# yjh0410/YOLO-Nano

Measured on NVIDIA B200. Metric: images/sec YOLO-Nano-1.0x 416 bs256 fp32-parity e2e (backbone+neck+head+decode+NMS), higher is better.
Workload: dtype f32 (tcgen05 3xTF32 split, fp32 accumulate)

## Files before the change

### yolo_nano_b200/csrc/ptx_sm100.cuh

```cuda
#pragma once
#include <cuda.h>
#include <cuda_runtime.h>
#include <stdint.h>

namespace ynb {
namespace ptx {

__device__ __forceinline__ uint32_t smem_u32(const void* p) {
  return (uint32_t)__cvta_generic_to_shared(p);
}

__device__ __forceinline__ void mbar_init(uint64_t* bar, uint32_t count) {
  asm volatile("mbarrier.init.shared::cta.b64 [%0], %1;" ::"r"(smem_u32(bar)), "r"(count));
}
__device__ __forceinline__ void fence_barrier_init() {
  asm volatile("fence.mbarrier_init.release.cluster;" ::: "memory");
}
__device__ __forceinline__ void mbar_arrive(uint64_t* bar) {
  asm volatile("mbarrier.arrive.shared::cta.b64 _, [%0];" ::"r"(smem_u32(bar)) : "memory");
}
__device__ __forceinline__ void mbar_arrive_expect_tx(uint64_t* bar, uint32_t bytes) {
  asm volatile("mbarrier.arrive.expect_tx.shared::cta.b64 _, [%0], %1;" ::"r"(smem_u32(bar)), "r"(bytes)
               : "memory");
}
// ... 26 lines not shown
  }
  if (timeout_flag) atomicCAS(timeout_flag, 0, code);
  return false;
}

__device__ __forceinline__ void fence_proxy_async_smem() {
  asm volatile("fence.proxy.async.shared::cta;" ::: "memory");
}
__device__ __forceinline__ void tc_fence_before_sync() {
  asm volatile("tcgen05.fence::before_thread_sync;" ::: "memory");
}
__device__ __forceinline__ void tc_fence_after_sync() {
  asm volatile("tcgen05.fence::after_thread_sync;" ::: "memory");
}

__device__ __forceinline__ void prefetch_tmap(const CUtensorMap* m) {
  asm volatile("prefetch.tensormap [%0];" ::"l"(reinterpret_cast<uint64_t>(m)) : "memory");
}
__device__ __forceinline__ void tma_load_2d(void* smem_dst, const CUtensorMap* m, uint64_t* bar, int c0, int c1) {
  asm volatile(
      "cp.async.bulk.tensor.2d.shared::cluster.global.mbarrier::complete_tx::bytes [%0], [%1, {%3, %4}], [%2];"
      ::"r"(smem_u32(smem_dst)), "l"(reinterpret_cast<uint64_t>(m)), "r"(smem_u32(bar)), "r"(c0), "r"(c1)
      : "memory");
}
__device__ __forceinline__ void tma_load_4d(void* smem_dst, const CUtensorMap* m, uint64_t* bar, int c0, int c1,
                                            int c2, int c3) {
  asm volatile(
      "cp.async.bulk.tensor.4d.shared::cluster.global.mbarrier::complete_tx::bytes [%0], [%1, {%3, %4, %5, %6}], [%2];"
      ::"r"(smem_u32(smem_dst)), "l"(reinterpret_cast<uint64_t>(m)), "r"(smem_u32(bar)), "r"(c0), "r"(c1),
      "r"(c2), "r"(c3)
      : "memory");
}

__device__ __forceinline__ void tma_prefetch_4d(const CUtensorMap* m, int c0, int c1, int c2, int c3) {
  asm volatile("cp.async.bulk.prefetch.tensor.4d.L2.global.tile [%0, {%1, %2, %3, %4}];"
               ::"l"(reinterpret_cast<uint64_t>(m)), "r"(c0), "r"(c1), "r"(c2), "r"(c3)
               : "memory");
}

__device__ __forceinline__ void cp_async_16(void* smem_dst, const void* gsrc, uint32_t src_bytes) {
  asm volatile("cp.async.cg.shared.global [%0], [%1], 16, %2;" ::"r"(smem_u32(smem_dst)), "l"(gsrc), "r"(src_bytes)
               : "memory");
}
__device__ __forceinline__ void cp_async_commit() { asm volatile("cp.async.commit_group;" ::: "memory"); }
__device__ __forceinline__ void cp_async_wait_all() { asm volatile("cp.async.wait_group 0;" ::: "memory"); }

__device__ __forceinline__ void tma_store_2d(const CUtensorMap* m, const void* smem_src, int c0, int c1) {
  asm volatile("cp.async.bulk.tensor.2d.global.shared::cta.bulk_group [%0, {%2, %3}], [%1];"
               ::"l"(reinterpret_cast<uint64_t>(m)), "r"(smem_u32(smem_src)), "r"(c0), "r"(c1)
               : "memory");
}
__device__ __forceinline__ void tma_store_4d(const CUtensorMap* m, const void* smem_src, int c0, int c1, int c2, int c3) {
  asm volatile("cp.async.bulk.tensor.4d.global.shared::cta.bulk_group [%0, {%2, %3, %4, %5}], [%1];"
               ::"l"(reinterpret_cast<uint64_t>(m)), "r"(smem_u32(smem_src)), "r"(c0), "r"(c1), "r"(c2), "r"(c3)
               : "memory");
}
__device__ __forceinline__ void bulk_commit() { asm volatile("cp.async.bulk.commit_group;" ::: "memory"); }
template <int N>
__device__ __forceinline__ void bulk_wait_read() {
  asm volatile("cp.async.bulk.wait_group.read %0;" ::"n"(N) : "memory");
}
template <int N>
__device__ __forceinline__ void bulk_wait() {
  asm volatile("cp.async.bulk.wait_group %0;" ::"n"(N) : "memory");
}

// ... 99 lines not shown
```

### yolo_nano_b200/csrc/unit_tc.cuh

```cuda
#pragma once
#include "gemm_tc.cuh"

namespace ynb {

constexpr int kDpThreads = 640;
constexpr int kDpEpiWarps = 8;
constexpr int kDpDwWarp0 = 8, kDpDwWarps = 8;
constexpr int kDpRawWarp = 16, kDpMmaWarp = 17, kDpWWarp = 18;
constexpr int kDpMaxAStages = 4, kDpMaxRawStages = 4;
constexpr int kDpStgBytes = kDpEpiWarps * 4096;

struct DwPwParams {
  int H, W, lgTW, tiles_x, tiles_y;
  int64_t num_tiles;
  int C4;
  int num_chunks;
  int ksub;
  int N, Npad;
  int mode;
  int w_resident, a_stages, raw_stages;
  int prefetch_tiles;
  int pass_blocks;
  int tma_out;
  uint32_t tmem_cols;
  const float* dw_w;
  const float* dw_b;
  int dw_act;
  float* out;
  int out_ld, out_off;
  ChanMap omap;
  const float* bias;
  int act;
  const float* pass;
  int pass_ld;
  int* err_flag;
  long long* trace;
};

#define YNB_DP_TRACE(role, lt, kc)                                                              \
  do {                                                                                           \
    if (p.trace != nullptr && blockIdx.x == 0 && (lt) < 16)                                      \
      p.trace[((role) * 16 + (lt)) * 8 + ((kc) & 7)] = clock64();                               \
  } while (0)

struct DpSmemLayout {
  uint32_t raw_stride, a_off, a_stride, w_chunk_bytes, w_res_off, dww_off, bias_off, stg_off, bar_off, total;
};

__host__ __device__ inline DpSmemLayout dp_smem_layout(int Npad, int num_chunks, int lgTW, int a_stages, int raw_stages,
                                                       bool w_resident, bool split, int chunk_ch = 32) {
  DpSmemLayout L;
  const int TW = 1 << lgTW, TH = kTcBM >> lgTW;
  L.w_chunk_bytes = (uint32_t)Npad * 128;
  L.raw_stride = ((uint32_t)((TW + 2) * (TH + 2) * 128) + 1023u) & ~1023u;
  L.a_off = L.raw_stride * raw_stages;
  L.a_stride = kTcAStageBytes * (split ? 2 : 1) + (w_resident ? 0 : L.w_chunk_bytes * (split ? 2 : 1));
  L.w_res_off = L.a_off + L.a_stride * a_stages;
  const uint32_t w_res = w_resident ? L.w_chunk_bytes * (split ? 2 : 1) * num_chunks : 0;
  L.dww_off = L.w_res_off + w_res;
  L.bias_off = L.dww_off + (((uint32_t)(10 * num_chunks * chunk_ch * 4) + 1023u) & ~1023u);
  L.stg_off = L.bias_off + 1024;
  L.bar_off = L.stg_off + kDpStgBytes;
  L.total = L.bar_off + 256 + 1024;
  return L;
}

__device__ __forceinline__ float cvt_rna_tf32(float x) {
  uint32_t r;
  asm("cvt.rna.tf32.f32 %0, %1;" : "=r"(r) : "f"(x));
  return __uint_as_float(r);
}

template <bool kPass, typename E>
__global__ void __launch_bounds__(kDpThreads, 1)
dwpw_tc_kernel(const __grid_constant__ CUtensorMap tmIn, const __grid_constant__ CUtensorMap tmWhi,
               const __grid_constant__ CUtensorMap tmWlo, const __grid_constant__ CUtensorMap tmPass,
               const __grid_constant__ CUtensorMap tmOut, const DwPwParams p) {
  extern __shared__ __align__(16) uint8_t smem_raw[];
  uint8_t* smem = smem_raw + ((1024u - (ptx::smem_u32(smem_raw) & 1023u)) & 1023u);

  constexpr bool kBf16 = sizeof(E) == 2;
  constexpr int CH = 128 / (int)sizeof(E);
  constexpr int CGS = CH / 4;
  const bool split = !kBf16 && p.mode == YNB_GEMM_TC_3XTF32;
  const DpSmemLayout lay = dp_smem_layout(p.Npad, p.num_chunks, p.lgTW, p.a_stages, p.raw_stages, p.w_resident != 0, split, CH);
  const uint32_t w_chunk_bytes = lay.w_chunk_bytes;
  const int KC = p.num_chunks * CH;
  const int TW = 1 << p.lgTW, TH = kTcBM >> p.lgTW;
  float* s_dww = reinterpret_cast<float*>(smem + lay.dww_off);
  float* s_bias = reinterpret_cast<float*>(smem + lay.bias_off);
  uint64_t* bars = reinterpret_cast<uint64_t*>(smem + lay.bar_off);
  uint64_t* raw_full = bars;
  uint64_t* raw_empty = bars + 4;
  uint64_t* a_ready = bars + 8;
  uint64_t* a_empty = bars + 12;
  uint64_t* w_full = bars + 16;
  uint64_t* tmem_full = bars + 20;
  uint64_t* tmem_empty = bars + 22;
  uint32_t* tmem_ptr = reinterpret_cast<uint32_t*>(bars + 24);

  const int warp = threadIdx.x >> 5, lane = threadIdx.x & 31;
  pdl_trigger();

  if (warp == kDpRawWarp && lane == 0) {
    ptx::prefetch_tmap(&tmIn);
    ptx::prefetch_tmap(&tmWhi);
    if (split) ptx::prefetch_tmap(&tmWlo);
    if (p.pass_blocks) ptx::prefetch_tmap(&tmPass);
    if (p.tma_out) ptx::prefetch_tmap(&tmOut);
    for (int s = 0; s < kDpMaxRawStages; ++s) {
      ptx::mbar_init(&raw_full[s], 1);
      ptx::mbar_init(&raw_empty[s], kBf16 ? kDpDwWarps : kDpDwWarps / 2);
    }
    for (int s = 0; s < kDpMaxAStages; ++s) {
      ptx::mbar_init(&a_ready[s], kBf16 ? kDpDwWarps : kDpDwWarps / 2);
      ptx::mbar_init(&a_empty[s], 1);
      ptx::mbar_init(&w_full[s], 1);
    }
// ... 9 lines not shown
  }
  for (int i = threadIdx.x; i < 10 * KC; i += kDpThreads) {
    const int tap = i / KC, c = i - tap * KC;
    float v = 0.0f;
    if (c < p.C4) v = tap < 9 ? __ldg(p.dw_w + tap * p.C4 + c) : __ldg(p.dw_b + c);
    s_dww[i] = v;
  }
  for (int i = threadIdx.x; i < p.Npad; i += kDpThreads) s_bias[i] = i < p.N ? __ldg(p.bias + i) : 0.0f;
  ptx::tc_fence_before_sync();
  __syncthreads();
  ptx::tc_fence_after_sync();
  const uint32_t tmem_base = *tmem_ptr;

  const int nacc = split ? 2 : 1;
  const int acc_cols = p.Npad * nacc;
  const int per_img = p.tiles_x * p.tiles_y;
  auto a_stage = [&](int s) { return smem + lay.a_off + (size_t)s * lay.a_stride; };
  auto w_hi_ptr = [&](int s, int kc) {
    return p.w_resident ? smem + lay.w_res_off + (size_t)kc * w_chunk_bytes * (split ? 2 : 1)
                        : a_stage(s) + kTcAStageBytes * (split ? 2 : 1);
  };

  if (warp == kDpRawWarp && p.w_resident && ptx::elect_one()) {
    ptx::mbar_arrive_expect_tx(&w_full[0], w_chunk_bytes * (split ? 2 : 1) * p.num_chunks);
    for (int kc = 0; kc < p.num_chunks; ++kc) {
      ptx::tma_load_2d(w_hi_ptr(0, kc), &tmWhi, &w_full[0], kc * CH, 0);
      if (split) ptx::tma_load_2d(w_hi_ptr(0, kc) + w_chunk_bytes, &tmWlo, &w_full[0], kc * CH, 0);
    }
  }
  pdl_wait();

  if (warp == kDpRawWarp) {
    if (ptx::elect_one()) {
      const uint32_t raw_bytes = (uint32_t)((TW + 2) * (TH + 2) * 128);
      int r = 0;
      uint32_t ph = 0;
      bool ok = true;
      for (int64_t tile = blockIdx.x; tile < p.num_tiles && ok; tile += gridDim.x) {
        const int b = (int)(tile / per_img);
        const int rr = (int)(tile - (int64_t)b * per_img);
        const int y0 = (rr / p.tiles_x) * TH, x0 = (rr % p.tiles_x) * TW;
#pragma unroll 1
        for (int cb = 0; cb < p.pass_blocks; ++cb) ptx::tma_prefetch_4d(&tmPass, cb * CH, x0, y0, b);
        if (p.prefetch_tiles > 0) {
          const int64_t tp = tile + (int64_t)p.prefetch_tiles * gridDim.x;
          if (tp < p.num_tiles) {
            const int bp = (int)(tp / per_img);
            const int rp = (int)(tp - (int64_t)bp * per_img);
            const int yp = (rp / p.tiles_x) * TH, xp = (rp % p.tiles_x) * TW;
#pragma unroll 1
            for (int kc = 0; kc < p.num_chunks; ++kc) ptx::tma_prefetch_4d(&tmIn, kc * CH, xp - 1, yp - 1, bp);
          }
        }
        for (int kc = 0; kc < p.num_chunks; ++kc) {
          ok = ptx::mbar_wait(&raw_empty[r], ph ^ 1, p.err_flag, 1);
          if (!ok) break;
          ptx::mbar_arrive_expect_tx(&raw_full[r], raw_bytes);
          ptx::tma_load_4d(smem + (size_t)r * lay.raw_stride, &tmIn, &raw_full[r], kc * CH, x0 - 1, y0 - 1, b);
          YNB_DP_TRACE(0, (int)((tile - blockIdx.x) / gridDim.x), kc);
          if (++r == p.raw_stages) { r = 0; ph ^= 1; }
        }
      }
    }
  } else if (warp == kDpWWarp) {
    if (!p.w_resident && ptx::elect_one()) {
      int s = 0;
      uint32_t ph = 0;
      bool ok = true;
      for (int64_t tile = blockIdx.x; tile < p.num_tiles && ok; tile += gridDim.x) {
        for (int kc = 0; kc < p.num_chunks; ++kc) {
          ok = ptx::mbar_wait(&a_empty[s], ph ^ 1, p.err_flag, 2);
// ... 34 lines not shown
          for (int k = 0; k < kTcBK / 8; ++k) {
            if (k >= nk) break;
            const uint32_t ko = k * 32;
            const uint32_t accum = (kc | k) != 0;
            const uint64_t da = ptx::make_sw128_kmajor_desc(a_hi + ko);
            const uint64_t db = ptx::make_sw128_kmajor_desc(b_hi + ko);
            if (kBf16) {
              ptx::mma_bf16_ss(d_tmem, da, db, idesc, accum);
            } else if (stack_b) {
              ptx::mma_tf32_ss(d_tmem, da, db, idesc2, accum);
              ptx::mma_tf32_ss(c_tmem, ptx::make_sw128_kmajor_desc(a_lo + ko), db, idesc, 1);
            } else if (split) {
              ptx::mma_tf32_ss(c_tmem, ptx::make_sw128_kmajor_desc(a_lo + ko), db, idesc, accum);
              ptx::mma_tf32_ss(c_tmem, da, ptx::make_sw128_kmajor_desc(b_lo + ko), idesc, 1);
              ptx::mma_tf32_ss(d_tmem, da, db, idesc, accum);
            } else {
              ptx::mma_tf32_ss(d_tmem, da, db, idesc, accum);
            }
          }
          YNB_DP_TRACE(3, (int)((tile - blockIdx.x) / gridDim.x), kc);
          ptx::mma_commit(&a_empty[s]);
          if (kc == p.num_chunks - 1) ptx::mma_commit(&tmem_full[acc]);
          if (++s == p.a_stages) { s = 0; ph ^= 1; }
        }
        if (++acc == 2) { acc = 0; acc_ph ^= 1; }
      }
    }
  } else if (warp >= kDpDwWarp0 && warp < kDpDwWarp0 + kDpDwWarps) {
    constexpr int NGROUPS = kBf16 ? 1 : 2;
    constexpr int GTHREADS = 256 / NGROUPS;
    const int t = (threadIdx.x - kDpDwWarp0 * 32) % GTHREADS;
    const int grp = (threadIdx.x - kDpDwWarp0 * 32) / GTHREADS;
    const int cg = t & (CGS - 1);
    const int IW = TW + 2;
    const bool has_act = p.dw_act != YNB_ACT_NONE;
    const float slope = p.dw_act == YNB_ACT_RELU ? 0.0f : 0.1f;
    const int nloc = (int64_t)blockIdx.x < p.num_tiles
                         ? (int)((p.num_tiles - blockIdx.x + gridDim.x - 1) / gridDim.x) : 0;
    const int total_chunks = nloc * p.num_chunks;
    bool ok = true;
    {
      for (int gc = grp; gc < total_chunks && ok; gc += NGROUPS) {
        const int lt_ = gc / p.num_chunks, kc = gc - lt_ * p.num_chunks;
        const int r = gc % p.raw_stages, s = gc % p.a_stages;
        const uint32_t rph = (uint32_t)((gc / p.raw_stages) & 1), sph = (uint32_t)((gc / p.a_stages) & 1);
        const float* wv = s_dww + kc * CH + cg * 4;
        const float4 bv = *reinterpret_cast<const float4*>(wv + 9 * KC);
        ok = ptx::mbar_wait(&raw_full[r], rph, p.err_flag, 7);
        if (ok) ok = ptx::mbar_wait(&a_empty[s], sph ^ 1, p.err_flag, 8);
        if (!ok) break;
        if (t == 0) YNB_DP_TRACE(1, lt_, kc);
        const uint8_t* raw = smem + (size_t)r * lay.raw_stride;
        uint8_t* a_hi = a_stage(s);
        uint8_t* a_lo = a_hi + kTcAStageBytes;
        constexpr int ROWS = 2;
        const int bidx = t / CGS;
        const int nsx = TW >> 2;
        const int sx = bidx % nsx, sy = (bidx / nsx) * ROWS;
        float4 acc[ROWS][4];
#pragma unroll
        for (int o = 0; o < ROWS; ++o)
#pragma unroll
          for (int q = 0; q < 4; ++q) acc[o][q] = bv;
#pragma unroll
        for (int ir = 0; ir < ROWS + 2; ++ir) {
          const int r0 = (sy + ir) * IW + sx * 4;
          float4 v[6];
#pragma unroll
          for (int j = 0; j < 6; ++j) {
            const int rr = r0 + j;
            if (!kBf16) v[j] = load4(reinterpret_cast<const E*>(raw + rr * 128 + (cg << 4)));
            else v[j] = load4(reinterpret_cast<const E*>(raw + rr * 128 + (cg << 3)));
          }
#pragma unroll
          for (int o = 0; o < ROWS; ++o) {
            const int ky = ir - o;
            if (ky < 0 || ky > 2) continue;
#pragma unroll
            for (int kx = 0; kx < 3; ++kx) {
              const float4 k = *reinterpret_cast<const float4*>(wv + (ky * 3 + kx) * KC);
#pragma unroll
              for (int q = 0; q < 4; ++q) {
                const float4 u = v[q + kx];
                const float2 lo = __ffma2_rn(make_float2(u.x, u.y), make_float2(k.x, k.y), make_float2(acc[o][q].x, acc[o][q].y));
                const float2 hi = __ffma2_rn(make_float2(u.z, u.w), make_float2(k.z, k.w), make_float2(acc[o][q].z, acc[o][q].w));
                acc[o][q] = make_float4(lo.x, lo.y, hi.x, hi.y);
              }
            }
          }
        }
        __syncwarp();
        if (lane == 0) ptx::mbar_arrive(&raw_empty[r]);
#pragma unroll
        for (int o = 0; o < ROWS; ++o) {
          const int row0 = (sy + o) * TW + sx * 4;
#pragma unroll
          for (int q = 0; q < 4; ++q) {
            const int row = row0 + q;
            float4 a = acc[o][q];
            if (has_act) {
              a.x = fmaxf(a.x, a.x * slope); a.y = fmaxf(a.y, a.y * slope);
              a.z = fmaxf(a.z, a.z * slope); a.w = fmaxf(a.w, a.w * slope);
            }
            if (kBf16) {
              const uint32_t o2 = (uint32_t)row * 128 + ((uint32_t)((cg >> 1) ^ (row & 7)) << 4) + ((uint32_t)(cg & 1) << 3);
              *reinterpret_cast<uint2*>(a_hi + o2) = make_uint2(pack_bf16x2(a.x, a.y), pack_bf16x2(a.z, a.w));
            } else {
              const uint32_t o2 = (uint32_t)row * 128 + ((uint32_t)(cg ^ (row & 7)) << 4);
              if (split) {
                float4 h, l;
                h.x = cvt_rna_tf32(a.x); h.y = cvt_rna_tf32(a.y); h.z = cvt_rna_tf32(a.z); h.w = cvt_rna_tf32(a.w);
                l.x = cvt_rna_tf32(a.x - h.x); l.y = cvt_rna_tf32(a.y - h.y);
                l.z = cvt_rna_tf32(a.z - h.z); l.w = cvt_rna_tf32(a.w - h.w);
                *reinterpret_cast<float4*>(a_hi + o2) = h;
                *reinterpret_cast<float4*>(a_lo + o2) = l;
              } else {
                *reinterpret_cast<float4*>(a_hi + o2) = a;
              }
            }
          }
        }
        ptx::fence_proxy_async_smem();
        __syncwarp();
        if (lane == 0) ptx::mbar_arrive(&a_ready[s]);
        if (t == 0) YNB_DP_TRACE(2, lt_, kc);
      }
    }
  } else if (warp < kDpEpiWarps) {
    const int group = warp >> 2, q = warp & 3;
    const int row = q * 32 + lane;
    const float slope = p.act == YNB_ACT_RELU ? 0.0f : (p.act == YNB_ACT_LEAKY ? 0.1f : 1.0f);
    uint8_t* sbox = smem + lay.stg_off + warp * 4096;
    const int sw = lane & 7;
    const int yy = row >> p.lgTW, xx = row & (TW - 1);
    const bool gap = p.omap.gap != 0;
    constexpr int BOX = 128 / (int)sizeof(E);
    constexpr int CPB = kPass ? BOX / 2 : BOX;
    constexpr int EPC = 16 / (int)sizeof(E);
    const int nbox = (p.Npad + CPB - 1) / CPB;
    const int out_cols = kPass ? 2 * p.N : ((p.N + EPC - 1) / EPC) * EPC;
    E* const outp = reinterpret_cast<E*>(p.out);
    const E* const passp = reinterpret_cast<const E*>(p.pass);
    const int acc = group;
    bool ok = true;
    int lt = group;
    for (int64_t tile = blockIdx.x + (int64_t)group * gridDim.x; tile < p.num_tiles && ok; tile += 2 * (int64_t)gridDim.x, lt += 2) {
      const uint32_t acc_ph = (uint32_t)((lt >> 1) & 1);
      const int b = (int)(tile / per_img);
      const int rr = (int)(tile - (int64_t)b * per_img);
      const int y = (rr / p.tiles_x) * TH + yy, x = (rr % p.tiles_x) * TW + xx;
      const bool valid = y < p.H && x < p.W;
      const int pix = (b * p.H + y) * p.W + x;
      const int ooff = valid ? pix * p.out_ld : -1;
      const E* prow = passp + (valid ? (size_t)pix * p.pass_ld : 0);
      uint4 x1v[4];
      auto fetch_x1 = [&](int c0) {
#pragma unroll
        for (int j = 0; j < 4; ++j)
          x1v[j] = (kPass && valid && c0 + EPC * j < p.N) ? __ldg(reinterpret_cast<const uint4*>(prow + c0) + j)
                                                         : make_uint4(0u, 0u, 0u, 0u);
      };
      if (kPass) fetch_x1(0);
      ok = ptx::mbar_wait(&tmem_full[acc], acc_ph, p.err_flag, 9);
      if (!ok) break;
      ptx::tc_fence_after_sync();
      if (q == 0 && lane == 0) YNB_DP_TRACE(4, lt, 0);
      const uint32_t t_base = tmem_base + ((uint32_t)(q * 32) << 16) + (uint32_t)(acc * acc_cols);
      auto drain16 = [&](int c0, float (&v)[16]) {
        uint32_t r1[16];
        ptx::tmem_ld_32x16(t_base + c0, r1);
        if (nacc == 2) {
          uint32_t r2[16];
          ptx::tmem_ld_32x16(t_base + (uint32_t)p.Npad + c0, r2);
          ptx::tmem_ld_wait();
#pragma unroll
          for (int j = 0; j < 16; ++j) v[j] = __uint_as_float(r1[j]) + __uint_as_float(r2[j]);
        } else {
          ptx::tmem_ld_wait();
#pragma unroll
          for (int j = 0; j < 16; ++j) v[j] = __uint_as_float(r1[j]);
        }
#pragma unroll
        for (int j = 0; j < 4; ++j) {
          const float4 b4 = *reinterpret_cast<const float4*>(s_bias + c0 + 4 * j);
          v[4 * j] += b4.x; v[4 * j + 1] += b4.y; v[4 * j + 2] += b4.z; v[4 * j + 3] += b4.w;
// ... 58 lines not shown
                const uint32_t x1bits = (i & 1) ? (xs >> 16) : (xs & 0xffffu);
                w[i] = x1bits | (pack_bf16x2(0.0f, v[i]) & 0xffff0000u);
              }
#pragma unroll
              for (int j = 0; j < 4; ++j) put_chunk(4 * h + j, make_uint4(w[4 * j], w[4 * j + 1], w[4 * j + 2], w[4 * j + 3]));
            }
          }
        } else {
          box_free();
#pragma unroll
          for (int h = 0; h < 4; ++h) {
            if (h == 0 || c0 + 16 * h < p.Npad) {
              float v[16];
              drain16(c0 + 16 * h, v);
              put_chunk(2 * h, make_uint4(pack_bf16x2(v[0], v[1]), pack_bf16x2(v[2], v[3]), pack_bf16x2(v[4], v[5]),
                                          pack_bf16x2(v[6], v[7])));
              put_chunk(2 * h + 1, make_uint4(pack_bf16x2(v[8], v[9]), pack_bf16x2(v[10], v[11]), pack_bf16x2(v[12], v[13]),
                                              pack_bf16x2(v[14], v[15])));
            }
          }
        }
        if (kPass && bx + 1 < nbox) fetch_x1((bx + 1) * CPB);
        if (bx == nbox - 1) {
          ptx::tc_fence_before_sync();
          __syncwarp();
          if (lane == 0) ptx::mbar_arrive(&tmem_empty[acc]);
        }
        __syncwarp();
        const int j0 = bx * BOX;
        if (tma_out) {
          ptx::fence_proxy_async_smem();
          __syncwarp();
          if (ptx::elect_one()) {
            ptx::tma_store_4d(&tmOut, sbox, j0, (rr % p.tiles_x) * TW, (rr / p.tiles_x) * TH + q * (32 >> p.lgTW), b);
            ptx::bulk_commit();
          }
          continue;
        }
        if (!gap) {
          const int ch = lane & 7;
          const int jc = j0 + EPC * ch;
#pragma unroll
          for (int k = 0; k < 8; ++k) {
            const int r = (lane >> 3) + 4 * k;
            const int oo = __shfl_sync(0xffffffffu, ooff, r);
            const uint4 val = *reinterpret_cast<const uint4*>(sbox + r * 128 + ((ch ^ (r & 7)) << 4));
            if (oo >= 0 && jc < out_cols) *reinterpret_cast<uint4*>(outp + oo + p.out_off + jc) = val;
          }
        } else if (!kBf16) {
          const int pr = lane & 15;
          const int jc = j0 + 2 * pr;
          const int col = p.omap.slot(p.out_off + jc);
#pragma unroll
          for (int k = 0; k < 16; ++k) {
            const int r = (lane >> 4) + 2 * k;
            const int oo = __shfl_sync(0xffffffffu, ooff, r);
            const uint2 val =
                *reinterpret_cast<const uint2*>(sbox + r * 128 + ((((pr >> 1) ^ (r & 7)) << 4) | ((pr & 1) << 3)));
            if (oo >= 0 && jc < out_cols) *reinterpret_cast<uint2*>(outp + oo + col) = val;
          }
        } else {
          const int jc = j0 + 2 * lane;
          const int col = p.omap.slot(p.out_off + jc);
#pragma unroll 8
          for (int r = 0; r < 32; ++r) {
            const int oo = __shfl_sync(0xffffffffu, ooff, r);
            const uint32_t val =
// ... 5 lines not shown
      }
      if (q == 0 && lane == 0) YNB_DP_TRACE(5, lt, 0);
    }
    if (p.tma_out && ptx::elect_one()) ptx::bulk_wait<0>();
  }

  ptx::tc_fence_before_sync();
  __syncthreads();
  if (warp == kDpMmaWarp) {
    ptx::tc_fence_after_sync();
    ptx::tmem_dealloc(tmem_base, p.tmem_cols);
  }
}

struct DwPwLaunch {
  CUtensorMap tmIn;
  CUtensorMap tmOut;
  CUtensorMap tmPass;
  const TcWeights* w = nullptr;
  DwPwParams p;
  uint32_t smem = 0;
  unsigned grid = 0;
};

inline bool plan_dwpw(DwPwLaunch& L, const void* in, int in_ld, int B, int H, int W, int C, int C4, const TcWeights* w,
                      int mode) {
  DwPwParams& p = L.p;
  const bool split = mode == YNB_GEMM_TC_3XTF32;
  const bool is_bf16 = mode == YNB_GEMM_TC_BF16;
  const int es = is_bf16 ? 2 : 4, chunk_ch = 128 / es;
  if (2 * (split ? 2 : 1) * w->Npad > 512 || (reinterpret_cast<uintptr_t>(in) & 15u) || ((in_ld * es) & 15)) return false;
  if ((int64_t)B * H * W * std::max(p.out_ld, std::max(p.pass_ld, 1)) >= (1LL << 31)) return false;
  p.H = H; p.W = W;
  {
    const int t16 = ((W + 15) / 16) * ((H + 7) / 8), t32 = ((W + 31) / 32) * ((H + 3) / 4);
    p.lgTW = t32 < t16 ? 5 : 4;
    static const int force = getenv("YNB_DP_LGTW") ? atoi(getenv("YNB_DP_LGTW")) : 0;
    if (force == 4 || force == 5) p.lgTW = force;
  }
  const int TW = 1 << p.lgTW, TH = kTcBM >> p.lgTW;
  p.tiles_x = (W + TW - 1) / TW;
  p.tiles_y = (H + TH - 1) / TH;
  p.num_tiles = (int64_t)B * p.tiles_x * p.tiles_y;
  p.C4 = C4;
  p.num_chunks = w->Kpad / chunk_ch;
  p.ksub = (C * es + 31) / 32;
  p.N = w->N; p.Npad = w->Npad;
  p.mode = mode;
  p.tmem_cols = 32;
  while ((int)p.tmem_cols < 2 * (split ? 2 : 1) * p.Npad) p.tmem_cols <<= 1;
  bool found = false;
  static const int wres = getenv("YNB_DP_WRES") ? atoi(getenv("YNB_DP_WRES")) : -1;
  for (int raw = kDpMaxRawStages; raw >= 2 && !found; --raw)
    for (int resident = 1; resident >= 0 && !found; --resident) {
      if (wres >= 0 && resident != wres) continue;
      DpSmemLayout lay = dp_smem_layout(p.Npad, p.num_chunks, p.lgTW, 2, raw, resident != 0, split, chunk_ch);
      if (lay.total <= (uint32_t)kTcSmemBudget) {
        p.a_stages = 2; p.raw_stages = raw; p.w_resident = resident; L.smem = lay.total;
        found = true;
      }
    }
  if (!found) return false;
  {
    static const int pf = getenv("YNB_DP_PREFETCH") ? atoi(getenv("YNB_DP_PREFETCH")) : 0;
    p.prefetch_tiles = pf;
  }
  const int epc = 16 / es;
  if ((reinterpret_cast<uintptr_t>(p.out) & 15u) || (p.out_ld % epc) || (p.out_off % epc)) return false;
  p.pass_blocks = 0;
  if (p.pass) {
    if ((reinterpret_cast<uintptr_t>(p.pass) & 15u) || (p.pass_ld % epc)) return false;
    if (make_tmap_nhwc(&L.tmPass, p.pass, (p.N + epc - 1) / epc * epc, W, H, B, p.pass_ld, TW, TH, is_bf16))
      p.pass_blocks = (p.N + chunk_ch - 1) / chunk_ch;
  }
  if (!make_tmap_nhwc(&L.tmIn, in, C4, W, H, B, in_ld, TW + 2, TH + 2, is_bf16, false)) return false;
  p.tma_out = 0;
  {
    static const bool no_ts = getenv("YNB_DP_NO_TMA_STORE") != nullptr;
    const int out_cols = p.pass ? 2 * p.N : (p.N + epc - 1) / epc * epc;
    if (!no_ts && p.omap.gap == 0 && p.out_off == 0 &&
        make_tmap_nhwc(&L.tmOut, p.out, out_cols, W, H, B, p.out_ld, TW, 32 / TW, is_bf16))
      p.tma_out = 1;
  }
  L.w = w;
  L.grid = (unsigned)std::min<int64_t>(p.num_tiles, kNumSMs);
  return true;
}

inline cudaError_t launch_dwpw_tc(const DwPwLaunch& L, cudaStream_t st) {
  using KernelT = void (*)(CUtensorMap, CUtensorMap, CUtensorMap, CUtensorMap, CUtensorMap, DwPwParams);
  static const KernelT kernels[4] = {dwpw_tc_kernel<false, float>, dwpw_tc_kernel<true, float>,
                                     dwpw_tc_kernel<false, bf16>, dwpw_tc_kernel<true, bf16>};
  static bool attr_set = false;
  if (!attr_set) {
    for (KernelT k : kernels) {
      cudaError_t e = cudaFuncSetAttribute(k, cudaFuncAttributeMaxDynamicSharedMemorySize, kTcSmemBudget);
      if (e != cudaSuccess) return e;
    }
    attr_set = true;
  }
  const int ki = (L.p.mode == YNB_GEMM_TC_BF16 ? 2 : 0) + (L.p.pass != nullptr ? 1 : 0);
  cudaError_t r = launch_pdl(kernels[ki], dim3(L.grid), dim3(kDpThreads), (size_t)L.smem, st,
                             L.tmIn, L.w->tm_hi, L.w->tm_lo, L.p.pass_blocks ? L.tmPass : L.tmIn,
                             L.p.tma_out ? L.tmOut : L.tmIn, L.p);
  YNB_COUNT_LAUNCH();
  return r;
}

}
```

### yolo_nano_b200/csrc/ynb_api.cu

```cuda
#include <cuda.h>
#include <cuda_runtime.h>

#include <cmath>
#include <cstdio>
#include <cstdlib>
#include <cstring>
#include <deque>
#include <functional>
#include <map>
#include <memory>
#include <string>
#include <tuple>
#include <vector>

#include "yolonano_b200.h"

#include "common.cuh"
#include "decode_nms.cuh"
#include "nms_grid.cuh"
#include "gemm_ffma.cuh"
#include "gemm_tc.cuh"
#include "unit_tc.cuh"
#include "kernels_basic.cuh"
#include "train_ops.cuh"
// ... 1611 lines not shown
  UNIT_TRY(cudaMemcpy(t.hi, hi.data(), hi.size() * 4, cudaMemcpyHostToDevice));
  UNIT_TRY(cudaMemcpy(t.lo, lo.data(), lo.size() * 4, cudaMemcpyHostToDevice));
  if (bfm) UNIT_TRY(cudaMemcpy(t.hi, bwv.data(), bwv.size() * 2, cudaMemcpyHostToDevice));
  int rc = YNB_OK;
  DwPwLaunch L;
  DwPwParams& p = L.p;
  memset(&p, 0, sizeof(p));
  p.dw_w = dw_w; p.dw_b = dw_b; p.dw_act = dw_act;
  p.out = out; p.out_ld = out_ld; p.out_off = 0; p.omap = dense_map();
  p.bias = pw_b; p.act = act; p.pass = pass; p.pass_ld = pass ? pass_ld : 0; p.err_flag = d_err;
  long long* d_trace = nullptr;
  const bool want_trace = getenv("YNB_DP_TRACE") != nullptr;
  if (want_trace) {
    UNIT_TRY(cudaMalloc(&d_trace, 6 * 16 * 8 * 8));
    UNIT_TRY(cudaMemset(d_trace, 0, 6 * 16 * 8 * 8));
    p.trace = d_trace;
  }
  if (!make_tmap_2d(&t.tm_hi, t.hi, t.Kpad, t.Npad, t.Kpad, t.Npad, bfm) ||
      !make_tmap_2d(&t.tm_lo, t.lo, t.Kpad, t.Npad, t.Kpad, t.Npad) ||
      !plan_dwpw(L, in, in_ld, batch, h, w_, channels, channels, &t, mode)) {
    rc = fail(nullptr, YNB_ERR_CUDA, "ynb_dwpw_tc: tensor map / smem planning failed");
  } else {
    cudaError_t r = launch_dwpw_tc(L, st);
    if (r == cudaSuccess) r = cudaStreamSynchronize(st);
    int flag = 0;
    if (r == cudaSuccess) r = cudaMemcpy(&flag, d_err, 4, cudaMemcpyDeviceToHost);
    if (r != cudaSuccess) rc = fail(nullptr, YNB_ERR_CUDA, std::string("ynb_dwpw_tc: ") + cudaGetErrorString(r));
    else if (flag) rc = fail(nullptr, YNB_ERR_CUDA, "ynb_dwpw_tc: mbarrier timeout code " + std::to_string(flag));
    if (want_trace && r == cudaSuccess) {
      std::vector<long long> h(6 * 16 * 8);
      cudaMemcpy(h.data(), d_trace, h.size() * 8, cudaMemcpyDeviceToHost);
      long long t0 = 0;
      for (long long v : h) if (v && (!t0 || v < t0)) t0 = v;
      fprintf(stderr, "YNB_DP_TRACE chunks=%d a_stages=%d raw_stages=%d resident=%d lgTW=%d tiles=%lld grid=%u\n", L.p.num_chunks,
              L.p.a_stages, L.p.raw_stages, L.p.w_resident, L.p.lgTW, (long long)L.p.num_tiles, L.grid);
      const char* names[6] = {"raw_issued", "raw_landed", "A_written", "mma_issued", "acc_ready", "epi_done"};
      for (int lt = 0; lt < 16; ++lt)
        for (int role = 0; role < 6; ++role) {
          std::string line;
          for (int kc = 0; kc < 8; ++kc)
            if (h[(role * 16 + lt) * 8 + kc]) line += " " + std::to_string(h[(role * 16 + lt) * 8 + kc] - t0);
          if (!line.empty()) fprintf(stderr, "TRACE tile %2d %-11s%s\n", lt, names[role], line.c_str());
        }
    }
  }
  if (d_trace) cudaFree(d_trace);
  cudaFree(t.hi); cudaFree(t.lo); cudaFree(d_err);
  return rc;
}

YNB_EXPORT int ynb_stem_pool(const float* x, float* out, const float* w, const float* b, int32_t batch,
                             int32_t input_size, void* stream) {
  if (!x || !out || !w || !b || input_size % 32) return fail(nullptr, YNB_ERR_INVALID, "ynb_stem_pool: bad arguments");
  StemWeights wt;
  UNIT_TRY(cudaMemcpy(wt.w, w, sizeof(wt.w), cudaMemcpyDeviceToHost));
  UNIT_TRY(cudaMemcpy(wt.b, b, sizeof(wt.b), cudaMemcpyDeviceToHost));
  CUtensorMap tmx{};
  const int use_tma = make_tmap_stem_input(&tmx, x, input_size, batch) ? 1 : 0;
  UNIT_TRY(launch_stem_pool(x, out, false, wt, tmx, use_tma, batch, input_size, (cudaStream_t)stream));
  return YNB_OK;
}

YNB_EXPORT int ynb_decode_level(const float* raw, int32_t raw_ld, float* boxes, float* scores, int32_t* cls,
                                int32_t batch, int32_t grid, int32_t stride_px, int32_t input_size,
                                const float* anchors_wh, int32_t num_anchors, int32_t num_classes,
                                int64_t boxes_per_image, int64_t level_off, void* stream) {
  if (!raw || !boxes || !scores || !cls || !anchors_wh || num_anchors > 4)
    return fail(nullptr, YNB_ERR_INVALID, "ynb_decode_level: bad arguments");
// ... 717 lines not shown
```

Measured before the change: 35230.

## Add flat pixel tiling to fused depthwise+pointwise tensor-core kernel

Adds a flat tiling mode in which each tile covers 128 consecutive pixels across the flattened B*H*W space, replacing 2D rectangular tiles when W is small enough. Raw input is loaded as a single 2D TMA box holding the tile plus one halo row above and below. Border taps are masked with per-thread bitmasks, and output and pass stores use 2D tensor maps. The goal is to remove the padding waste of rectangular tiles on small or odd feature maps and cut tile count. In exchange it adds halo rows spanning full image width, larger raw smem stages, and extra per-tap branching in the depthwise loop.

After: 35240, median of 6. No clear change (+0.0%).

```diff
diff --git a/yolo_nano_b200/csrc/ptx_sm100.cuh b/yolo_nano_b200/csrc/ptx_sm100.cuh
--- a/yolo_nano_b200/csrc/ptx_sm100.cuh
+++ b/yolo_nano_b200/csrc/ptx_sm100.cuh
@@ -82,6 +82,11 @@
       : "memory");
 }
 
+__device__ __forceinline__ void tma_prefetch_2d(const CUtensorMap* m, int c0, int c1) {
+  asm volatile("cp.async.bulk.prefetch.tensor.2d.L2.global.tile [%0, {%1, %2}];"
+               ::"l"(reinterpret_cast<uint64_t>(m)), "r"(c0), "r"(c1)
+               : "memory");
+}
 __device__ __forceinline__ void tma_prefetch_4d(const CUtensorMap* m, int c0, int c1, int c2, int c3) {
   asm volatile("cp.async.bulk.prefetch.tensor.4d.L2.global.tile [%0, {%1, %2, %3, %4}];"
                ::"l"(reinterpret_cast<uint64_t>(m)), "r"(c0), "r"(c1), "r"(c2), "r"(c3)
diff --git a/yolo_nano_b200/csrc/unit_tc.cuh b/yolo_nano_b200/csrc/unit_tc.cuh
--- a/yolo_nano_b200/csrc/unit_tc.cuh
+++ b/yolo_nano_b200/csrc/unit_tc.cuh
@@ -12,6 +12,8 @@
 
 struct DwPwParams {
   int H, W, lgTW, tiles_x, tiles_y;
+  int flat;
+  int P;
   int64_t num_tiles;
   int C4;
   int num_chunks;
@@ -47,12 +49,17 @@
   uint32_t raw_stride, a_off, a_stride, w_chunk_bytes, w_res_off, dww_off, bias_off, stg_off, bar_off, total;
 };
 
-__host__ __device__ inline DpSmemLayout dp_smem_layout(int Npad, int num_chunks, int lgTW, int a_stages, int raw_stages,
-                                                       bool w_resident, bool split, int chunk_ch = 32) {
+constexpr int kDpFlatMaxW = (256 - kTcBM - 2) / 2;
+__host__ __device__ inline uint32_t dp_raw_box_bytes(int flat, int lgTW, int W) {
+  if (flat) return (uint32_t)(kTcBM + 2 * W + 2) * 128u;
+  return (uint32_t)(((1 << lgTW) + 2) * ((kTcBM >> lgTW) + 2) * 128);
+}
+
+__host__ __device__ inline DpSmemLayout dp_smem_layout(int Npad, int num_chunks, int flat, int lgTW, int W, int a_stages,
+                                                       int raw_stages, bool w_resident, bool split, int chunk_ch = 32) {
   DpSmemLayout L;
-  const int TW = 1 << lgTW, TH = kTcBM >> lgTW;
   L.w_chunk_bytes = (uint32_t)Npad * 128;
-  L.raw_stride = ((uint32_t)((TW + 2) * (TH + 2) * 128) + 1023u) & ~1023u;
+  L.raw_stride = (dp_raw_box_bytes(flat, lgTW, W) + 1023u) & ~1023u;
   L.a_off = L.raw_stride * raw_stages;
   L.a_stride = kTcAStageBytes * (split ? 2 : 1) + (w_resident ? 0 : L.w_chunk_bytes * (split ? 2 : 1));
   L.w_res_off = L.a_off + L.a_stride * a_stages;
@@ -83,7 +90,8 @@
   constexpr int CH = 128 / (int)sizeof(E);
   constexpr int CGS = CH / 4;
   const bool split = !kBf16 && p.mode == YNB_GEMM_TC_3XTF32;
-  const DpSmemLayout lay = dp_smem_layout(p.Npad, p.num_chunks, p.lgTW, p.a_stages, p.raw_stages, p.w_resident != 0, split, CH);
+  const DpSmemLayout lay =
+      dp_smem_layout(p.Npad, p.num_chunks, p.flat, p.lgTW, p.W, p.a_stages, p.raw_stages, p.w_resident != 0, split, CH);
   const uint32_t w_chunk_bytes = lay.w_chunk_bytes;
   const int KC = p.num_chunks * CH;
   const int TW = 1 << p.lgTW, TH = kTcBM >> p.lgTW;
@@ -159,11 +167,31 @@
 
   if (warp == kDpRawWarp) {
     if (ptx::elect_one()) {
-      const uint32_t raw_bytes = (uint32_t)((TW + 2) * (TH + 2) * 128);
+      const uint32_t raw_bytes = dp_raw_box_bytes(p.flat, p.lgTW, p.W);
       int r = 0;
       uint32_t ph = 0;
       bool ok = true;
-      for (int64_t tile = blockIdx.x; tile < p.num_tiles && ok; tile += gridDim.x) {
+      for (int64_t tile = blockIdx.x; tile < p.num_tiles && ok && p.flat; tile += gridDim.x) {
+        const int p0 = (int)tile * kTcBM;
+#pragma unroll 1
+        for (int cb = 0; cb < p.pass_blocks; ++cb) ptx::tma_prefetch_2d(&tmPass, cb * CH, p0);
+        if (p.prefetch_tiles > 0) {
+          const int64_t tp = tile + (int64_t)p.prefetch_tiles * gridDim.x;
+          if (tp < p.num_tiles) {
+#pragma unroll 1
+            for (int kc = 0; kc < p.num_chunks; ++kc) ptx::tma_prefetch_2d(&tmIn, kc * CH, (int)tp * kTcBM - p.W - 1);
+          }
+        }
+        for (int kc = 0; kc < p.num_chunks; ++kc) {
+          ok = ptx::mbar_wait(&raw_empty[r], ph ^ 1, p.err_flag, 1);
+          if (!ok) break;
+          ptx::mbar_arrive_expect_tx(&raw_full[r], raw_bytes);
+          ptx::tma_load_2d(smem + (size_t)r * lay.raw_stride, &tmIn, &raw_full[r], kc * CH, p0 - p.W - 1);
+          YNB_DP_TRACE(0, (int)((tile - blockIdx.x) / gridDim.x), kc);
+          if (++r == p.raw_stages) { r = 0; ph ^= 1; }
+        }
+      }
+      for (int64_t tile = blockIdx.x; tile < p.num_tiles && ok && !p.flat; tile += gridDim.x) {
         const int b = (int)(tile / per_img);
         const int rr = (int)(tile - (int64_t)b * per_img);
         const int y0 = (rr / p.tiles_x) * TH, x0 = (rr % p.tiles_x) * TW;
@@ -264,20 +292,30 @@
     const int t = (threadIdx.x - kDpDwWarp0 * 32) % GTHREADS;
     const int grp = (threadIdx.x - kDpDwWarp0 * 32) / GTHREADS;
     const int cg = t & (CGS - 1);
-    const int IW = TW + 2;
-    const bool has_act = p.dw_act != YNB_ACT_NONE;
-    const float slope = p.dw_act == YNB_ACT_RELU ? 0.0f : 0.1f;
-    const int nloc = (int64_t)blockIdx.x < p.num_tiles
-                         ? (int)((p.num_tiles - blockIdx.x + gridDim.x - 1) / gridDim.x) : 0;
-    const int total_chunks = nloc * p.num_chunks;
+    const int bidx = t / CGS;
+    uint32_t hbits = 0, vbits = 0;
     bool ok = true;
     {
-      for (int gc = grp; gc < total_chunks && ok; gc += NGROUPS) {
+      for (int gc = grp; ok; gc += NGROUPS) {
         const int lt_ = gc / p.num_chunks, kc = gc - lt_ * p.num_chunks;
+        if (blockIdx.x + (int64_t)lt_ * gridDim.x >= p.num_tiles) break;
         const int r = gc % p.raw_stages, s = gc % p.a_stages;
         const uint32_t rph = (uint32_t)((gc / p.raw_stages) & 1), sph = (uint32_t)((gc / p.a_stages) & 1);
         const float* wv = s_dww + kc * CH + cg * 4;
-        const float4 bv = *reinterpret_cast<const float4*>(wv + 9 * KC);
+        if (p.flat && kc < NGROUPS) {
+          const int p0 = (int)(blockIdx.x + (int64_t)lt_ * gridDim.x) * kTcBM;
+          const int ps = p0 + 8 * bidx;
+          const int g = ps / p.W;
+          int x = ps - g * p.W, y = g % p.H;
+          if (--x < 0) { x = p.W - 1; if (--y < 0) y = p.H - 1; }
+          hbits = vbits = 0;
+#pragma unroll
+          for (int m = 0; m < 10; ++m) {
+            vbits |= (uint32_t)(y == 0) << m | (uint32_t)(y == p.H - 1) << (16 + m);
+            if (m >= 1 && m <= 8) hbits |= (uint32_t)(x == 0) << (m - 1) | (uint32_t)(x == p.W - 1) << (7 + m);
+            if (++x == p.W) { x = 0; if (++y == p.H) y = 0; }
+          }
+        }
         ok = ptx::mbar_wait(&raw_full[r], rph, p.err_flag, 7);
         if (ok) ok = ptx::mbar_wait(&a_empty[s], sph ^ 1, p.err_flag, 8);
         if (!ok) break;
@@ -285,72 +323,98 @@
         const uint8_t* raw = smem + (size_t)r * lay.raw_stride;
         uint8_t* a_hi = a_stage(s);
         uint8_t* a_lo = a_hi + kTcAStageBytes;
-        constexpr int ROWS = 2;
-        const int bidx = t / CGS;
-        const int nsx = TW >> 2;
-        const int sx = bidx % nsx, sy = (bidx / nsx) * ROWS;
-        float4 acc[ROWS][4];
-#pragma unroll
-        for (int o = 0; o < ROWS; ++o)
-#pragma unroll
-          for (int q = 0; q < 4; ++q) acc[o][q] = bv;
-#pragma unroll
-        for (int ir = 0; ir < ROWS + 2; ++ir) {
-          const int r0 = (sy + ir) * IW + sx * 4;
-          float4 v[6];
-#pragma unroll
-          for (int j = 0; j < 6; ++j) {
-            const int rr = r0 + j;
-            if (!kBf16) v[j] = load4(reinterpret_cast<const E*>(raw + rr * 128 + (cg << 4)));
-            else v[j] = load4(reinterpret_cast<const E*>(raw + rr * 128 + (cg << 3)));
-          }
-#pragma unroll
-          for (int o = 0; o < ROWS; ++o) {
-            const int ky = ir - o;
-            if (ky < 0 || ky > 2) continue;
-#pragma unroll
-            for (int kx = 0; kx < 3; ++kx) {
-              const float4 k = *reinterpret_cast<const float4*>(wv + (ky * 3 + kx) * KC);
-#pragma unroll
-              for (int q = 0; q < 4; ++q) {
-                const float4 u = v[q + kx];
-                const float2 lo = __ffma2_rn(make_float2(u.x, u.y), make_float2(k.x, k.y), make_float2(acc[o][q].x, acc[o][q].y));
-                const float2 hi = __ffma2_rn(make_float2(u.z, u.w), make_float2(k.z, k.w), make_float2(acc[o][q].z, acc[o][q].w));
-                acc[o][q] = make_float4(lo.x, lo.y, hi.x, hi.y);
+        const int cgo = kBf16 ? (cg << 3) : (cg << 4);
+        auto tap = [&](float4& a, const float4 u, const float4 k) {
+          const float2 lo = __ffma2_rn(make_float2(u.x, u.y), make_float2(k.x, k.y), make_float2(a.x, a.y));
+          const float2 hi = __ffma2_rn(make_float2(u.z, u.w), make_float2(k.z, k.w), make_float2(a.z, a.w));
+          a = make_float4(lo.x, lo.y, hi.x, hi.y);
+        };
+        auto store_row = [&](int row, float4 a) {
+          if (p.dw_act != YNB_ACT_NONE) {
+            const float slope = p.dw_act == YNB_ACT_RELU ? 0.0f : 0.1f;
+            a.x = fmaxf(a.x, a.x * slope); a.y = fmaxf(a.y, a.y * slope);
+            a.z = fmaxf(a.z, a.z * slope); a.w = fmaxf(a.w, a.w * slope);
+          }
+          if (kBf16) {
+            const uint32_t o2 = (uint32_t)row * 128 + ((uint32_t)((cg >> 1) ^ (row & 7)) << 4) + ((uint32_t)(cg & 1) << 3);
+            *reinterpret_cast<uint2*>(a_hi + o2) = make_uint2(pack_bf16x2(a.x, a.y), pack_bf16x2(a.z, a.w));
+          } else {
+            const uint32_t o2 = (uint32_t)row * 128 + ((uint32_t)(cg ^ (row & 7)) << 4);
+            if (split) {
+              float4 h, l;
+              h.x = cvt_rna_tf32(a.x); h.y = cvt_rna_tf32(a.y); h.z = cvt_rna_tf32(a.z); h.w = cvt_rna_tf32(a.w);
+              l.x = cvt_rna_tf32(a.x - h.x); l.y = cvt_rna_tf32(a.y - h.y);
+              l.z = cvt_rna_tf32(a.z - h.z); l.w = cvt_rna_tf32(a.w - h.w);
+              *reinterpret_cast<float4*>(a_hi + o2) = h;
+              *reinterpret_cast<float4*>(a_lo + o2) = l;
+            } else {
+              *reinterpret_cast<float4*>(a_hi + o2) = a;
+            }
+          }
+        };
+        if (p.flat) {
+          const uint8_t* rb = raw + (8 * bidx + p.W) * 128 + cgo;
+#pragma unroll 1
+          for (int h = 0; h < 2; ++h) {
+            float4 acc[4];
+#pragma unroll
+            for (int q = 0; q < 4; ++q) acc[q] = *reinterpret_cast<const float4*>(wv + 9 * KC);
+#pragma unroll 1
+            for (int ky = 0; ky < 3; ++ky) {
+              const uint8_t* rrow = rb + ((ptrdiff_t)(ky - 1) * p.W + 4 * h) * 128;
+              const uint32_t vskip = (ky == 0 ? vbits : (ky == 2 ? vbits >> 16 : 0u)) >> (4 * h + 1);
+              float4 v[6];
+#pragma unroll
+              for (int m = 0; m < 6; ++m) v[m] = load4(reinterpret_cast<const E*>(rrow + m * 128));
+#pragma unroll
+              for (int kx = 0; kx < 3; ++kx) {
+                const uint32_t skip = vskip | ((kx == 0 ? hbits : (kx == 2 ? hbits >> 8 : 0u)) >> (4 * h));
+                const float4 k = *reinterpret_cast<const float4*>(wv + (ky * 3 + kx) * KC);
+#pragma unroll
+                for (int q = 0; q < 4; ++q)
+                  if (!((skip >> q) & 1)) tap(acc[q], v[q + kx], k);
               }
             }
-          }
-        }
-        __syncwarp();
-        if (lane == 0) ptx::mbar_arrive(&raw_empty[r]);
-#pragma unroll
-        for (int o = 0; o < ROWS; ++o) {
-          const int row0 = (sy + o) * TW + sx * 4;
-#pragma unroll
-          for (int q = 0; q < 4; ++q) {
-            const int row = row0 + q;
-            float4 a = acc[o][q];
-            if (has_act) {
-              a.x = fmaxf(a.x, a.x * slope); a.y = fmaxf(a.y, a.y * slope);
-              a.z = fmaxf(a.z, a.z * slope); a.w = fmaxf(a.w, a.w * slope);
+            if (h == 1) {
+              __syncwarp();
+              if (lane == 0) ptx::mbar_arrive(&raw_empty[r]);
             }
-            if (kBf16) {
-              const uint32_t o2 = (uint32_t)row * 128 + ((uint32_t)((cg >> 1) ^ (row & 7)) << 4) + ((uint32_t)(cg & 1) << 3);
-              *reinterpret_cast<uint2*>(a_hi + o2) = make_uint2(pack_bf16x2(a.x, a.y), pack_bf16x2(a.z, a.w));
-            } else {
-              const uint32_t o2 = (uint32_t)row * 128 + ((uint32_t)(cg ^ (row & 7)) << 4);
-              if (split) {
-                float4 h, l;
-                h.x = cvt_rna_tf32(a.x); h.y = cvt_rna_tf32(a.y); h.z = cvt_rna_tf32(a.z); h.w = cvt_rna_tf32(a.w);
-                l.x = cvt_rna_tf32(a.x - h.x); l.y = cvt_rna_tf32(a.y - h.y);
-                l.z = cvt_rna_tf32(a.z - h.z); l.w = cvt_rna_tf32(a.w - h.w);
-                *reinterpret_cast<float4*>(a_hi + o2) = h;
-                *reinterpret_cast<float4*>(a_lo + o2) = l;
-              } else {
-                *reinterpret_cast<float4*>(a_hi + o2) = a;
+#pragma unroll
+            for (int q = 0; q < 4; ++q) store_row(8 * bidx + 4 * h + q, acc[q]);
+          }
+        } else {
+          const int nsx = TW >> 2;
+          const int sx = bidx % nsx, sy = (bidx / nsx) * 2;
+          const float4 bv = *reinterpret_cast<const float4*>(wv + 9 * KC);
+          float4 acc[2][4];
+#pragma unroll
+          for (int o = 0; o < 2; ++o)
+#pragma unroll
+            for (int q = 0; q < 4; ++q) acc[o][q] = bv;
+#pragma unroll
+          for (int ir = 0; ir < 4; ++ir) {
+            const int r0 = (sy + ir) * (TW + 2) + sx * 4;
+            float4 v[6];
+#pragma unroll
+            for (int j = 0; j < 6; ++j) v[j] = load4(reinterpret_cast<const E*>(raw + (r0 + j) * 128 + cgo));
+#pragma unroll
+            for (int o = 0; o < 2; ++o) {
+              const int ky = ir - o;
+              if (ky < 0 || ky > 2) continue;
+#pragma unroll
+              for (int kx = 0; kx < 3; ++kx) {
+                const float4 k = *reinterpret_cast<const float4*>(wv + (ky * 3 + kx) * KC);
+#pragma unroll
+                for (int q = 0; q < 4; ++q) tap(acc[o][q], v[q + kx], k);
               }
             }
           }
+          __syncwarp();
+          if (lane == 0) ptx::mbar_arrive(&raw_empty[r]);
+#pragma unroll
+          for (int o = 0; o < 2; ++o)
+#pragma unroll
+            for (int q = 0; q < 4; ++q) store_row((sy + o) * TW + sx * 4 + q, acc[o][q]);
         }
         ptx::fence_proxy_async_smem();
         __syncwarp();
@@ -378,11 +442,18 @@
     int lt = group;
     for (int64_t tile = blockIdx.x + (int64_t)group * gridDim.x; tile < p.num_tiles && ok; tile += 2 * (int64_t)gridDim.x, lt += 2) {
       const uint32_t acc_ph = (uint32_t)((lt >> 1) & 1);
-      const int b = (int)(tile / per_img);
-      const int rr = (int)(tile - (int64_t)b * per_img);
-      const int y = (rr / p.tiles_x) * TH + yy, x = (rr % p.tiles_x) * TW + xx;
-      const bool valid = y < p.H && x < p.W;
-      const int pix = (b * p.H + y) * p.W + x;
+      int b = 0, rr = 0, pix;
+      bool valid;
+      if (p.flat) {
+        pix = (int)tile * kTcBM + row;
+        valid = pix < p.P;
+      } else {
+        b = (int)(tile / per_img);
+        rr = (int)(tile - (int64_t)b * per_img);
+        const int y = (rr / p.tiles_x) * TH + yy, x = (rr % p.tiles_x) * TW + xx;
+        valid = y < p.H && x < p.W;
+        pix = (b * p.H + y) * p.W + x;
+      }
       const int ooff = valid ? pix * p.out_ld : -1;
       const E* prow = passp + (valid ? (size_t)pix * p.pass_ld : 0);
       uint4 x1v[4];
@@ -507,7 +578,10 @@
           ptx::fence_proxy_async_smem();
           __syncwarp();
           if (ptx::elect_one()) {
-            ptx::tma_store_4d(&tmOut, sbox, j0, (rr % p.tiles_x) * TW, (rr / p.tiles_x) * TH + q * (32 >> p.lgTW), b);
+            if (p.flat)
+              ptx::tma_store_2d(&tmOut, sbox, j0, (int)tile * kTcBM + q * 32);
+            else
+              ptx::tma_store_4d(&tmOut, sbox, j0, (rr % p.tiles_x) * TW, (rr / p.tiles_x) * TH + q * (32 >> p.lgTW), b);
             ptx::bulk_commit();
           }
           continue;
@@ -579,6 +653,7 @@
   if (2 * (split ? 2 : 1) * w->Npad > 512 || (reinterpret_cast<uintptr_t>(in) & 15u) || ((in_ld * es) & 15)) return false;
   if ((int64_t)B * H * W * std::max(p.out_ld, std::max(p.pass_ld, 1)) >= (1LL << 31)) return false;
   p.H = H; p.W = W;
+  p.P = B * H * W;
   {
     const int t16 = ((W + 15) / 16) * ((H + 7) / 8), t32 = ((W + 31) / 32) * ((H + 3) / 4);
     p.lgTW = t32 < t16 ? 5 : 4;
@@ -588,7 +663,7 @@
   const int TW = 1 << p.lgTW, TH = kTcBM >> p.lgTW;
   p.tiles_x = (W + TW - 1) / TW;
   p.tiles_y = (H + TH - 1) / TH;
-  p.num_tiles = (int64_t)B * p.tiles_x * p.tiles_y;
+  const int64_t rect_tiles = (int64_t)B * p.tiles_x * p.tiles_y, flat_tiles = ((int64_t)p.P + kTcBM - 1) / kTcBM;
   p.C4 = C4;
   p.num_chunks = w->Kpad / chunk_ch;
   p.ksub = (C * es + 31) / 32;
@@ -596,35 +671,59 @@
   p.mode = mode;
   p.tmem_cols = 32;
   while ((int)p.tmem_cols < 2 * (split ? 2 : 1) * p.Npad) p.tmem_cols <<= 1;
-  bool found = false;
   static const int wres = getenv("YNB_DP_WRES") ? atoi(getenv("YNB_DP_WRES")) : -1;
-  for (int raw = kDpMaxRawStages; raw >= 2 && !found; --raw)
-    for (int resident = 1; resident >= 0 && !found; --resident) {
-      if (wres >= 0 && resident != wres) continue;
-      DpSmemLayout lay = dp_smem_layout(p.Npad, p.num_chunks, p.lgTW, 2, raw, resident != 0, split, chunk_ch);
-      if (lay.total <= (uint32_t)kTcSmemBudget) {
-        p.a_stages = 2; p.raw_stages = raw; p.w_resident = resident; L.smem = lay.total;
-        found = true;
+  auto plan_smem = [&](int flat) {
+    for (int raw = kDpMaxRawStages; raw >= 2; --raw)
+      for (int resident = 1; resident >= 0; --resident) {
+        if (wres >= 0 && resident != wres) continue;
+        DpSmemLayout lay = dp_smem_layout(p.Npad, p.num_chunks, flat, p.lgTW, W, 2, raw, resident != 0, split, chunk_ch);
+        if (lay.total <= (uint32_t)kTcSmemBudget) {
+          p.a_stages = 2; p.raw_stages = raw; p.w_resident = resident; L.smem = lay.total;
+          return true;
+        }
       }
-    }
-  if (!found) return false;
+    return false;
+  };
   {
     static const int pf = getenv("YNB_DP_PREFETCH") ? atoi(getenv("YNB_DP_PREFETCH")) : 0;
     p.prefetch_tiles = pf;
   }
   const int epc = 16 / es;
   if ((reinterpret_cast<uintptr_t>(p.out) & 15u) || (p.out_ld % epc) || (p.out_off % epc)) return false;
+  if (p.pass && ((reinterpret_cast<uintptr_t>(p.pass) & 15u) || (p.pass_ld % epc))) return false;
+  const int pass_cols = (p.N + epc - 1) / epc * epc;
+  const int out_cols = p.pass ? 2 * p.N : (p.N + epc - 1) / epc * epc;
+  static const bool no_ts = getenv("YNB_DP_NO_TMA_STORE") != nullptr;
+  const char* rect_env = getenv("YNB_DP_RECT");
+  const bool force_rect = rect_env != nullptr && atoi(rect_env) != 0;
+  p.flat = 0;
+  const int rect_resident = plan_smem(0) ? p.w_resident : 0;
+  if (!force_rect && !no_ts && p.omap.gap == 0 && p.out_off == 0 && W <= kDpFlatMaxW && flat_tiles < rect_tiles &&
+      plan_smem(1) && p.w_resident >= rect_resident) {
+    PFN_encodeTiled enc = get_encode_tiled();
+    const cuuint64_t dims[2] = {(cuuint64_t)C4, (cuuint64_t)p.P};
+    const cuuint64_t strides[1] = {(cuuint64_t)in_ld * es};
+    const cuuint32_t box[2] = {(cuuint32_t)chunk_ch, (cuuint32_t)(kTcBM + 2 * W + 2)};
+    const cuuint32_t estr[2] = {1, 1};
+    p.flat = enc &&
+             enc(&L.tmIn, is_bf16 ? CU_TENSOR_MAP_DATA_TYPE_BFLOAT16 : CU_TENSOR_MAP_DATA_TYPE_FLOAT32, 2,
+                 const_cast<void*>(in), dims, strides, box, estr, CU_TENSOR_MAP_INTERLEAVE_NONE, CU_TENSOR_MAP_SWIZZLE_NONE,
+                 CU_TENSOR_MAP_L2_PROMOTION_L2_128B, CU_TENSOR_MAP_FLOAT_OOB_FILL_NONE) == CUDA_SUCCESS &&
+             make_tmap_2d(&L.tmOut, p.out, out_cols, p.P, p.out_ld, 32, is_bf16);
+  }
   p.pass_blocks = 0;
-  if (p.pass) {
-    if ((reinterpret_cast<uintptr_t>(p.pass) & 15u) || (p.pass_ld % epc)) return false;
-    if (make_tmap_nhwc(&L.tmPass, p.pass, (p.N + epc - 1) / epc * epc, W, H, B, p.pass_ld, TW, TH, is_bf16))
+  p.tma_out = 0;
+  if (p.flat) {
+    p.num_tiles = flat_tiles;
+    p.tma_out = 1;
+    if (p.pass && make_tmap_2d(&L.tmPass, p.pass, pass_cols, p.P, p.pass_ld, kTcBM, is_bf16))
       p.pass_blocks = (p.N + chunk_ch - 1) / chunk_ch;
-  }
-  if (!make_tmap_nhwc(&L.tmIn, in, C4, W, H, B, in_ld, TW + 2, TH + 2, is_bf16, false)) return false;
-  p.tma_out = 0;
-  {
-    static const bool no_ts = getenv("YNB_DP_NO_TMA_STORE") != nullptr;
-    const int out_cols = p.pass ? 2 * p.N : (p.N + epc - 1) / epc * epc;
+  } else {
+    p.num_tiles = rect_tiles;
+    if (!plan_smem(0)) return false;
+    if (p.pass && make_tmap_nhwc(&L.tmPass, p.pass, pass_cols, W, H, B, p.pass_ld, TW, TH, is_bf16))
+      p.pass_blocks = (p.N + chunk_ch - 1) / chunk_ch;
+    if (!make_tmap_nhwc(&L.tmIn, in, C4, W, H, B, in_ld, TW + 2, TH + 2, is_bf16, false)) return false;
     if (!no_ts && p.omap.gap == 0 && p.out_off == 0 &&
         make_tmap_nhwc(&L.tmOut, p.out, out_cols, W, H, B, p.out_ld, TW, 32 / TW, is_bf16))
       p.tma_out = 1;
diff --git a/yolo_nano_b200/csrc/ynb_api.cu b/yolo_nano_b200/csrc/ynb_api.cu
--- a/yolo_nano_b200/csrc/ynb_api.cu
+++ b/yolo_nano_b200/csrc/ynb_api.cu
@@ -1667,8 +1667,8 @@
       cudaMemcpy(h.data(), d_trace, h.size() * 8, cudaMemcpyDeviceToHost);
       long long t0 = 0;
       for (long long v : h) if (v && (!t0 || v < t0)) t0 = v;
-      fprintf(stderr, "YNB_DP_TRACE chunks=%d a_stages=%d raw_stages=%d resident=%d lgTW=%d tiles=%lld grid=%u\n", L.p.num_chunks,
-              L.p.a_stages, L.p.raw_stages, L.p.w_resident, L.p.lgTW, (long long)L.p.num_tiles, L.grid);
+      fprintf(stderr, "YNB_DP_TRACE chunks=%d a_stages=%d raw_stages=%d resident=%d flat=%d lgTW=%d tiles=%lld grid=%u smem=%u\n", L.p.num_chunks,
+              L.p.a_stages, L.p.raw_stages, L.p.w_resident, L.p.flat, L.p.lgTW, (long long)L.p.num_tiles, L.grid, L.smem);
       const char* names[6] = {"raw_issued", "raw_landed", "A_written", "mma_issued", "acc_ready", "epi_done"};
       for (int lt = 0; lt < 16; ++lt)
         for (int role = 0; role < 6; ++role) {
```
